# innate2adaptive/decombinator

Measured on AMD Instinct MI355X. Metric: Mreads/s decombined (150 bp human-beta), higher is better.
Workload: dtype u8

## Files before the change

decombinator_amd/csrc/dcrx_kernels_v2.hip:

```cpp
#include <hip/hip_runtime.h>
#include <hip/hip_ext.h>

#include <algorithm>
#include <cstddef>
#include <cstdio>
#include <cstdlib>
#include <vector>

#include "../../include/dcrx.h"
#include "dcrx_device.h"
#include "dcrx_launch.h"
#include "dcrx_dcr_device.h"
#include "dcrx_v2_device.h"
#include "dcrx_sink_device.h"

namespace dcrx {

bool first_use_on_device(bool (&seen)[64]);
void attributes_set_on_device(bool (&seen)[64]);

constexpr int DCRX_V2_BLOCK = 1024;
#ifdef DCRX_SCAN_STAMPS
__device__ uint32_t *g_scan_stamps;
#endif
constexpr int DCRX_V2_FBLOCK = 256;
#ifndef DCRX_V2_TBLOCK
#define DCRX_V2_TBLOCK 256
#define DCRX_V2_TWAVES 5
#endif
// ... 12 lines not shown
#define DCRX_STORE_SCAN dcrx_store_record_cached
#else
#define DCRX_STORE_SCAN dcrx_store_record
#endif
#ifndef DCRX_V2_LOOP_PRIO
#define DCRX_V2_LOOP_PRIO 2
#endif
#ifndef DCRX_V2_FULL_LINE_RECORDS
#define DCRX_V2_FULL_LINE_RECORDS 1
#endif
#ifndef DCRX_V2_ROLE_CALLS
#define DCRX_V2_ROLE_CALLS 0
#endif
#if DCRX_V2_ROLE_CALLS
#define DCRX_V2_ROLE __device__ __attribute__((noinline))
#else
#define DCRX_V2_ROLE __device__ __forceinline__
#endif
#ifndef DCRX_LEAN_LDS_WORDS
#define DCRX_LEAN_LDS_WORDS 1
#endif
constexpr uint32_t DCRX_V2_GROUP_MAX = 64;

enum { V2_L_TAIL = 0, V2_L_E = 1, V2_L_C = 2, V2_L_X = 3, V2_L_RING = 4, V2_L_TICKETS = 5, V2_L_TWHINT = 6, V2_L_COUNTS = 8 };
constexpr uint32_t V2_LEFT_CAP = 1024;
enum { V2_QC_LEFT = 5, V2_QC_DONE = 6 };
struct V2Lists {
  uint4 *tail;
  uint4 *ev;
  uint4 *sx;
  uint4 *left;
  uint32_t *counts;
  uint32_t tcap, ecap, scap;
};
template <int NW>
struct V2Rows {
  static constexpr int T = (2 + NW + 3) / 4, E = (1 + 2 * NW + 3) / 4;
  static_assert((2 + 2 * NW + 3) / 4 == E, "the digest word of an event entry (put_event) lies in the entry's last row");
};
struct V2ListRef { uint4 *rows; uint32_t cap; };
template <int NW>
__device__ __forceinline__ V2ListRef v2_list(const V2Lists &Q, const int which, const size_t region) {
  constexpr size_t E = V2Rows<NW>::E;
  if (which == V2_L_E) return V2ListRef{Q.ev + region * Q.ecap * E, Q.ecap};
  return V2ListRef{Q.sx + (region * Q.scap + (which == V2_L_X ? Q.scap / 2 : 0u)) * E, Q.scap / 2};
}
template <int N>
// ... 162 lines not shown
  for (uint64_t i = (uint64_t)e_lo + (uint32_t)tid; i < e_hi; i += blockDim.x) {
    const uint32_t r = B.exc_read[i];
    if (set) { if (i == e_lo || B.exc_read[i - 1] != r) atomicOr(&flag[r >> 5], 1u << (r & 31)); }
    else flag[r >> 5] = 0u;
  }
}

template <int NW>
__device__ __forceinline__ uint32_t *v2_left_valid(uint4 *left_rows) { return reinterpret_cast<uint32_t *>(left_rows + (size_t)V2_LEFT_CAP * V2Rows<NW>::E); }
template <int NW>
__device__ __forceinline__ bool v2_left_push(uint4 *left_rows, uint32_t *__restrict__ queue_count, const uint32_t x0, const uint32_t (&lg)[NW], const uint32_t (&w)[NW]) {
  const uint32_t at = atomicAdd(queue_count + V2_QC_LEFT, 1u);
  if (at >= V2_LEFT_CAP) return false;
  uint32_t x[1 + 2 * NW];
  x[0] = x0;
#pragma unroll
  for (int k = 0; k < NW; k++) { x[1 + k] = lg[k]; x[1 + NW + k] = w[k]; }
  v2_put_rows<1 + 2 * NW>(left_rows, 0u, at, x);
  __threadfence();
  __hip_atomic_store(v2_left_valid<NW>(left_rows) + at, 1u, __ATOMIC_RELAXED, __HIP_MEMORY_SCOPE_AGENT);
  return true;
}

enum { V2_WK_NEXT = 0, V2_WK_LIST = 1, V2_WK_EXC = 8, V2_WK_HEAD = 16, V2_WK_CLAIM = 17, V2_WK_SCANNED = 18, V2_WK_SINK = 19, V2_WK_HEAD2 = 20, V2_WK_CLAIM2 = 21,
       V2_WK_FILLED = 32, V2_WK_GEN = 48, V2_WK_FILLED2 = 64, V2_WK_GEN2 = 80, V2_WK_WORDS = 96 };
#ifndef DCRX_V2_FUSE_TAILWAVES
#define DCRX_V2_FUSE_TAILWAVES 3
#endif
#ifndef DCRX_V2_PRIO_TAIL
#define DCRX_V2_PRIO_TAIL 1
#endif
constexpr int V2_FUSE_TAILWAVES = DCRX_V2_FUSE_TAILWAVES;
constexpr uint32_t V2_TW6_FRAC256 = 243, V2_TW5_FRAC256 = 205, V2_TW4_FRAC256 = 136, V2_TW3_FRAC256 = 64;
constexpr int V2_RING_STRIDE = 15;
constexpr uint32_t V2_RING_MAXBATCHES = 16;
template <int NW> constexpr int v2_ering_stride() { return (2 * NW + 4) | 1; }
constexpr uint32_t V2_ERING_BATCHES = 8;
#ifndef DCRX_V2_HELP_DRAIN
#define DCRX_V2_HELP_DRAIN 0
#endif
constexpr float V2_FUSE_E_MAX_SHARE = 0.25f;

template <bool UNIFORM_LEN, int NW, int RPL, bool NARROW, bool PREFETCH = true, int FUSE = -1, bool SINK = false, bool FUSE_E = false>
__global__ __launch_bounds__(DCRX_V2_BLOCK) void scan2_kernel(
    DevTables T0, BatchDev B, CfgDev cfg, dcrx_record_t *__restrict__ records, unsigned long long *__restrict__ counters,
    V2Lists Q, uint32_t *__restrict__ queue, uint32_t *__restrict__ gqueue, uint32_t qcap, uint32_t *__restrict__ queue_count,
    uint64_t per_block, uint32_t retry, const DevTables *__restrict__ Tmem, uint32_t ring_batches, V2SinkCall S, uint32_t tail_waves, uint32_t rescue_waves) {
  static_assert(!FUSE_E || (FUSE >= 0 && !SINK), "the event ring rides on the fused form, without a tuple sink");
  extern __shared__ __align__(64) uint32_t smem[];
  if constexpr (FUSE >= 0 && !SINK) S.dev = nullptr;
  const int o = FUSE >= 0 ? FUSE : (cfg.orientation == DCRX_ORIENT_FORWARD ? 0 : 1);
  V2Ori V0 = T0.v2[0];
  if (o) V0 = T0.v2[1];
  uint32_t *lds_trans = smem;
  uint32_t *lds_counts = smem + V0.trans_bytes / 4;
  uint32_t *lds_work = lds_counts + DCRX_N_COUNTERS;
  const int tid = threadIdx.x;
#ifdef DCRX_SCAN_STAMPS
  const unsigned long long stamp_r0 = __builtin_amdgcn_s_memrealtime();
  unsigned long long stamp_setup = 0, stamp_loop_end = 0;
#endif
  if (tid < DCRX_N_COUNTERS) lds_counts[tid] = 0;
  if (tid < V2_WK_WORDS) lds_work[tid] = 0;
  {
    const uint4 *src = reinterpret_cast<const uint4 *>(V0.trans);
    uint4 *dst = reinterpret_cast<uint4 *>(lds_trans);
    for (uint32_t i = tid; i < V0.trans_bytes / 16; i += blockDim.x) dst[i] = src[i];
  }
  const V2Tab tab{};
  uint32_t *lds_side = lds_work + V2_WK_WORDS;
  uint32_t *lds_bk = lds_side + (T0.lds_image_bytes - T0.dfa_bytes) / 4;
  uint32_t *ring = lds_bk + V0.bk_bytes / 4;
  const uint32_t ring_mask = 64u * ring_batches - 1u;
  constexpr uint32_t ES = (uint32_t)v2_ering_stride<NW>(), ering_mask = 64u * V2_ERING_BATCHES - 1u;
  uint32_t *ring2 = ring + (size_t)(ring_mask + 1u) * V2_RING_STRIDE;
  uint32_t *lds_dry = ring2 + (size_t)(ering_mask + 1u) * ES;
  if (FUSE >= 0) {
    {
      const uint4 *s1 = reinterpret_cast<const uint4 *>(T0.image + T0.dfa_bytes), *s2 = reinterpret_cast<const uint4 *>(V0.bk);
      uint4 *d1 = reinterpret_cast<uint4 *>(lds_side), *d2 = reinterpret_cast<uint4 *>(lds_bk);
      for (uint32_t i = tid; i < (T0.lds_image_bytes - T0.dfa_bytes) / 16; i += blockDim.x) d1[i] = s1[i];
      for (uint32_t i = tid; i < V0.bk_bytes / 16; i += blockDim.x) d2[i] = s2[i];
    }
    for (uint32_t i = tid; i <= ring_mask; i += blockDim.x) { ring[i * V2_RING_STRIDE + NW] = 0u; ring[i * V2_RING_STRIDE + NW + 1] = 0u; }
    if (FUSE_E) for (uint32_t i = tid; i <= ering_mask; i += blockDim.x) { ring2[i * ES + NW] = 0u; ring2[i * ES + NW + 1] = 0u; }
  }
  __syncthreads();
  const uint32_t nw = B.stride >> 2;
  const int lane = tid & 63;
  const unsigned long long lt_mask = (1ull << lane) - 1ull;
  const bool tagged = B.n_reads < (1ull << 30);

  const uint64_t blk_lo = (uint64_t)blockIdx.x * per_block;
  const uint64_t blk_hi = blk_lo + per_block < B.n_reads ? blk_lo + per_block : B.n_reads;
  uint32_t e_lo = 0u, e_hi = 0u;
  if (B.n_exc) {
    v2_exc_slice(B, blk_lo < blk_hi ? blk_lo : blk_hi, blk_hi, lds_work + V2_WK_EXC, tid);
    e_lo = lds_work[V2_WK_EXC]; e_hi = lds_work[V2_WK_EXC + 2];
    v2_exc_marks(B, e_lo, e_hi, true, tid);
    asm volatile("s_waitcnt vmcnt(0)" ::: "memory");
    __syncthreads();
  }
  uint32_t tw = tail_waves;
  if (FUSE >= 0 && tw == 0u) {
    const uint32_t h = Q.counts[V2_L_COUNTS * blockIdx.x + V2_L_TWHINT + (o ? 0 : 1)];
    tw = (h >= 2u && h <= 8u) ? h : (uint32_t)V2_FUSE_TAILWAVES;
    if (FUSE_E && tw > 2u) tw -= 1u;
  }
// ... 103 lines not shown
        base = (uint32_t)__builtin_amdgcn_readfirstlane((int)base);
        const uint32_t at = base + (uint32_t)__popcll(mt0 & lt_mask);
        if (to_tail && at >= Q.tcap) { v2_hand_over(B, queue, gqueue, qcap, queue_count, tagged, (uint32_t)r, false); to_tail = false; }
        if (to_tail) {
          uint32_t x[2 + NW];
          x[0] = (uint32_t)r; x[1] = tail2_pack(d);
#pragma unroll
          for (int k = 0; k < NW; k++) x[2 + k] = w[q][k];
          v2_put_rows<2 + NW>(tq, Q.tcap, at, x);
        }
      }
      int lst = 0;
      if (what == V2_EVENTS) lst = (exc || bnd) ? V2_L_X : (shape2(d.vf_n, d.jf_n, d.any) == V2_SHAPE_BOTH ? V2_L_C : V2_L_E);
      auto put_event = [&](uint4 *rows, const uint32_t at) {
        uint32_t x[2 + 2 * NW];
        x[0] = (uint32_t)r | (exc ? V2_R_EXC : 0u);
#pragma unroll
        for (int k = 0; k < NW; k++) { x[1 + k] = lg[q][k]; x[1 + NW + k] = w[q][k]; }
        x[1 + 2 * NW] = rescue2_digest_pack(d);
        v2_put_rows<2 + 2 * NW>(rows, 0u, at, x);
      };
      bool to_ev = lst == V2_L_E;
      const unsigned long long me0 = __ballot(to_ev);
      if (FUSE_E) {
        if (me0) {
          constexpr uint32_t nb_mask = V2_ERING_BATCHES - 1u, nb_shift = (uint32_t)__builtin_ctz(V2_ERING_BATCHES);
          const uint32_t total = (uint32_t)__popcll(me0);
          const uint32_t genv = __hip_atomic_load(&lds_work[V2_WK_GEN2 + ((uint32_t)lane & nb_mask)], __ATOMIC_RELAXED, __HIP_MEMORY_SCOPE_WORKGROUP);
          uint32_t base = 0;
          if (lane == 0) base = atomicAdd(&lds_work[V2_WK_HEAD2], total);
          base = (uint32_t)__builtin_amdgcn_readfirstlane((int)base);
          const uint32_t gb0 = base >> 6, gbl = (base + total - 1u) >> 6;
          bool room = true;
          for (uint32_t g = gb0; g <= gbl; g++) room = room && (uint32_t)__builtin_amdgcn_readlane((int)genv, (int)(g & nb_mask)) >= (g >> nb_shift);
          if (!room && lane == 0) {
            bool ok = false;
            for (uint32_t spins = 0; spins < (1u << 24) && !ok; spins++) {
              ok = true;
              for (uint32_t g = gb0; g <= gbl; g++)
                ok = ok && __hip_atomic_load(&lds_work[V2_WK_GEN2 + (g & nb_mask)], __ATOMIC_RELAXED, __HIP_MEMORY_SCOPE_WORKGROUP) >= (g >> nb_shift);
              if (!ok) __builtin_amdgcn_s_sleep(2);
            }
            if (!ok) atomicAdd(&counters[DCRX_C_DEVICE_ERRORS], 1ull);
          }
          asm volatile("" ::: "memory");
          if (to_ev) {
            uint32_t *sl = ring2 + ((base + (uint32_t)__popcll(me0 & lt_mask)) & ering_mask) * ES;
#pragma unroll
            for (int k = 0; k < NW; k++) { sl[k] = w[q][k]; sl[NW + 3 + k] = lg[q][k]; }
            sl[NW + 2] = (uint32_t)r; sl[2 * NW + 3] = rescue2_digest_pack(d);
          }
          asm volatile("" ::: "memory");
          if (lane == 0) {
            for (uint32_t g = gb0; g <= gbl; g++) {
              const uint32_t lo = max(base, g << 6), hi = min(base + total, (g + 1u) << 6);
              atomicAdd(&lds_work[V2_WK_FILLED2 + (g & nb_mask)], hi - lo);
            }
          }
        }
      } else if (me0) {
        uint32_t base = 0;
        if (lane == 0) base = atomicAdd(&lds_work[V2_WK_LIST + V2_L_E], (uint32_t)__popcll(me0));
        base = (uint32_t)__builtin_amdgcn_readfirstlane((int)base);
        const uint32_t at = base + (uint32_t)__popcll(me0 & lt_mask);
        if (to_ev && at >= Q.ecap) {
          v2_hand_over(B, queue, gqueue, qcap, queue_count, tagged, (uint32_t)r, exc);
          to_ev = false;
        }
        if (to_ev) put_event(eq, at);
      }
      if (__ballot(lst > V2_L_E)) {
#pragma unroll 1
        for (int which = V2_L_C; which <= V2_L_X; which++) {
          const bool mine = lst == which;
          const unsigned long long mr = __ballot(mine);
          if (!mr) continue;
          uint32_t base = 0;
          if (lane == 0) base = atomicAdd(&lds_work[V2_WK_LIST + which], (uint32_t)__popcll(mr));
          base = (uint32_t)__builtin_amdgcn_readfirstlane((int)base);
          if (mine) {
            const V2ListRef l = v2_list<NW>(Q, which, region);
// ... 55 lines not shown
        for (int k = 0; k < NW; k++) w[q][k] = wn[q][k];
        xm[q] = xn[q];
      }
    }
    item = next;
  }
  if (FUSE >= 0 && lane == 0) {
    asm volatile("s_waitcnt lgkmcnt(0)" ::: "memory");
    atomicAdd(&lds_work[V2_WK_SCANNED], 1u);
  }
  }
  if (FUSE_E && (wv >= n_scan_waves + tw || (DCRX_V2_HELP_DRAIN && scans))) {
   if constexpr (FUSE_E) {
    constexpr bool REV = FUSE == 1;
#if DCRX_V2_PRIO_TAIL
    __builtin_amdgcn_s_setprio(DCRX_V2_PRIO_TAIL);
#endif
    uint32_t kw_base[K_NCLASS];
#pragma unroll
    for (int c = 0; c < K_NCLASS; c++) kw_base[c] = T0.kw_base[c];
    const Rescue2Tabs rt = rescue2_tabs(T0, V0, reinterpret_cast<const uint8_t *>(lds_side), reinterpret_cast<const uint8_t *>(lds_bk), REV, kw_base);
    const Counters C{lds_counts}, Cdry{lds_dry};
    constexpr uint32_t nb_mask = V2_ERING_BATCHES - 1u, nb_shift = (uint32_t)__builtin_ctz(V2_ERING_BATCHES);
    constexpr uint32_t V2_RING_EXIT = 0xFFFFFFFFu;
    for (uint32_t spins = 0;;) {
      uint32_t c = 0, nvalid = 0;
      if (lane == 0) {
        c = __hip_atomic_load(&lds_work[V2_WK_CLAIM2], __ATOMIC_RELAXED, __HIP_MEMORY_SCOPE_WORKGROUP);
        const bool mine = __hip_atomic_load(&lds_work[V2_WK_GEN2 + (c & nb_mask)], __ATOMIC_RELAXED, __HIP_MEMORY_SCOPE_WORKGROUP) == (c >> nb_shift);
        const uint32_t f = __hip_atomic_load(&lds_work[V2_WK_FILLED2 + (c & nb_mask)], __ATOMIC_RELAXED, __HIP_MEMORY_SCOPE_WORKGROUP);
        if (!mine) nvalid = 0;
        else if (f == 64u) nvalid = 64u;
        else if (__hip_atomic_load(&lds_work[V2_WK_SCANNED], __ATOMIC_RELAXED, __HIP_MEMORY_SCOPE_WORKGROUP) == n_scan_waves) {
          const uint32_t h = __hip_atomic_load(&lds_work[V2_WK_HEAD2], __ATOMIC_RELAXED, __HIP_MEMORY_SCOPE_WORKGROUP);
          const uint32_t rem = h - 64u * c;
          nvalid = (int32_t)rem <= 0 ? V2_RING_EXIT : min(rem, 64u);
        }
        if (nvalid && nvalid != V2_RING_EXIT) {
          uint32_t expect = c;
          if (!__hip_atomic_compare_exchange_strong(&lds_work[V2_WK_CLAIM2], &expect, c + 1u, __ATOMIC_RELAXED, __ATOMIC_RELAXED, __HIP_MEMORY_SCOPE_WORKGROUP)) nvalid = 0;
        }
      }
      c = (uint32_t)__builtin_amdgcn_readfirstlane((int)c);
      nvalid = (uint32_t)__builtin_amdgcn_readfirstlane((int)nvalid);
      if (nvalid == V2_RING_EXIT) break;
      if (!nvalid) {
        if (++spins > (1u << 24)) { if (lane == 0) atomicAdd(&counters[DCRX_C_DEVICE_ERRORS], 1ull); break; }
        __builtin_amdgcn_s_sleep(4);
        continue;
      }
      asm volatile("s_waitcnt lgkmcnt(0)" ::: "memory");
      uint32_t *sl = ring2 + ((64u * c + (uint32_t)lane) & ering_mask) * ES;
      int status = -2;
      uint32_t errs = 0, x0 = 0;
      uint32_t lg[NW];
#pragma unroll
      for (int k = 0; k < NW; k++) lg[k] = 0u;
      if ((uint32_t)lane < nvalid) {
        x0 = sl[NW + 2];
#pragma unroll
        for (int k = 0; k < NW; k++) lg[k] = sl[NW + 3 + k];
        const uint32_t dg = sl[2 * NW + 3];
        const uint32_t r = x0 & V2_R_MASK;
        const int n = UNIFORM_LEN ? (int)B.read_len : (int)B.lens[r];
        const LdsWords lw{dcrx_ldsaddr_of(sl)};
        auto on_ok = [&](dcrx_record_t rec, const uint32_t) {
          rec.frame = (uint8_t)(o ? 0 : 1);
          DCRX_STORE_FINISH(records + r, rec);
        };
        status = rescue2_fast_to<REV, NW, V2_SHAPE_ONE>(rt, lw, lg, n, cfg, on_ok, errs, *Tmem, C, Cdry, dg);
        if (status > 0) {
          dcrx_record_t rec;
          rec.v = rec.j = rec.v_start = rec.j_end = rec.ins_start = rec.ins_len = 0; rec.vdel = rec.jdel = 0;
          rec.status = (uint8_t)status; rec.frame = (uint8_t)(o ? 0 : 1);
          DCRX_STORE_FINISH(records + r, rec);
        } else if (status < 0) errs = 0;
      }
      v2_tally_rescue(lds_counts, lane, status, errs, o == 0);
      if (__builtin_expect(status == RESCUE2_SLOW, 0)) {
        uint32_t ww[NW];
#pragma unroll
        for (int k = 0; k < NW; k++) ww[k] = sl[k];
        if (!v2_left_push<NW>(Q.left, queue_count, x0, lg, ww)) v2_hand_over(B, queue, gqueue, qcap, queue_count, tagged, x0 & V2_R_MASK, false);
      }
      asm volatile("s_waitcnt lgkmcnt(0)" ::: "memory");
      if (lane == 0) {
        __hip_atomic_store(&lds_work[V2_WK_FILLED2 + (c & nb_mask)], 0u, __ATOMIC_RELAXED, __HIP_MEMORY_SCOPE_WORKGROUP);
        asm volatile("s_waitcnt lgkmcnt(0)" ::: "memory");
        atomicAdd(&lds_work[V2_WK_GEN2 + (c & nb_mask)], 1u);
      }
      spins = 0;
    }
   }
  }
  if (FUSE >= 0 && (DCRX_V2_HELP_DRAIN || (wv >= n_scan_waves && wv < n_scan_waves + tw))) {
   if constexpr (FUSE >= 0) {
    constexpr bool REV = FUSE == 1;
#if DCRX_V2_PRIO_TAIL
    __builtin_amdgcn_s_setprio(DCRX_V2_PRIO_TAIL);
#endif
    const Tail2Tabs tt = tail2_tabs(T0, V0, reinterpret_cast<const uint8_t *>(lds_side), reinterpret_cast<const uint8_t *>(lds_bk), REV);
    const Counters C{lds_counts};
    const uint32_t nb_mask = ring_batches - 1u, nb_shift = (uint32_t)__builtin_ctz(ring_batches);
    constexpr uint32_t V2_RING_EXIT = 0xFFFFFFFFu;
    for (uint32_t spins = 0;;) {
      uint32_t c = 0, nvalid = 0;
      if (lane == 0) {
        c = __hip_atomic_load(&lds_work[V2_WK_CLAIM], __ATOMIC_RELAXED, __HIP_MEMORY_SCOPE_WORKGROUP);
        const bool mine = __hip_atomic_load(&lds_work[V2_WK_GEN + (c & nb_mask)], __ATOMIC_RELAXED, __HIP_MEMORY_SCOPE_WORKGROUP) == (c >> nb_shift);
        const uint32_t f = __hip_atomic_load(&lds_work[V2_WK_FILLED + (c & nb_mask)], __ATOMIC_RELAXED, __HIP_MEMORY_SCOPE_WORKGROUP);
        if (!mine) nvalid = 0;
        else if (f == 64u) nvalid = 64u;
        else if (__hip_atomic_load(&lds_work[V2_WK_SCANNED], __ATOMIC_RELAXED, __HIP_MEMORY_SCOPE_WORKGROUP) == n_scan_waves) {
// ... 57 lines not shown
        __hip_atomic_store(&lds_work[V2_WK_FILLED + (c & nb_mask)], 0u, __ATOMIC_RELAXED, __HIP_MEMORY_SCOPE_WORKGROUP);
        asm volatile("s_waitcnt lgkmcnt(0)" ::: "memory");
        atomicAdd(&lds_work[V2_WK_GEN + (c & nb_mask)], 1u);
      }
      spins = 0;
    }
   }
  }
#ifdef DCRX_SCAN_STAMPS
  stamp_loop_end = __builtin_amdgcn_s_memrealtime();
#endif
  __syncthreads();
  if (B.n_exc) v2_exc_marks(B, e_lo, e_hi, false, tid);
#ifdef DCRX_SCAN_STAMPS
  if (lane == 0) {
    uint32_t *c = g_scan_stamps + 4 * ((size_t)blockIdx.x * (DCRX_V2_BLOCK / 64) + (size_t)(tid >> 6));
    c[0] = (uint32_t)stamp_r0; c[1] = (uint32_t)stamp_setup; c[2] = (uint32_t)stamp_loop_end; c[3] = (uint32_t)__builtin_amdgcn_s_memrealtime();
  }
#else
  if (tid < V2_L_COUNTS) {
    uint32_t c = tid <= V2_L_X ? lds_work[V2_WK_LIST + tid] : 0u;
    c = min(c, tid == V2_L_TAIL ? Q.tcap : (tid == V2_L_E ? Q.ecap : Q.scap / 2));
    if (tid == V2_L_RING) c = lds_work[V2_WK_HEAD];
    if ((tid == V2_L_TWHINT || tid == V2_L_TWHINT + 1) && FUSE >= 0) c = Q.counts[V2_L_COUNTS * region + tid];
    if (tid == V2_L_TWHINT + (o ? 0 : 1) && FUSE >= 0 && blk_hi > blk_lo) {
      const uint32_t frac256 = (uint32_t)(((uint64_t)lds_work[V2_WK_HEAD] << 8) / (blk_hi - blk_lo));
      c = frac256 >= V2_TW6_FRAC256 ? 6u : (frac256 >= V2_TW5_FRAC256 ? 5u : (frac256 >= V2_TW4_FRAC256 ? 4u : (frac256 >= V2_TW3_FRAC256 ? 3u : 2u)));
    }
    Q.counts[V2_L_COUNTS * region + tid] = c;
  }
  if (S.dev && tid == 0 && lds_work[V2_WK_SINK]) (void)__hip_atomic_fetch_add(S.hits + region, lds_work[V2_WK_SINK], __ATOMIC_RELAXED, __HIP_MEMORY_SCOPE_AGENT);
#endif
  if (tid < DCRX_N_COUNTERS && lds_counts[tid]) atomicAdd(&counters[tid], (unsigned long long)lds_counts[tid]);
}

static uint32_t v2_finish_lds_bytes(const DevTables &T, int o) {
  return DCRX_N_COUNTERS * 4 + (T.lds_image_bytes - T.dfa_bytes) + T.v2[o].bk_bytes;
}

template <bool UNIFORM_LEN, int NW, int ORI>
__device__ __forceinline__ void v2_general_entry(const DevTables &T, const V2Ori &V, const BatchDev &B, const CfgDev &cfg, const uint32_t x0,
                                                 const uint32_t (&lg)[NW], const uint32_t (&w)[NW], const Counters &C, dcrx_record_t *__restrict__ records,
                                                 uint32_t *__restrict__ queue, uint32_t *__restrict__ gqueue, const uint32_t qcap,
                                                 uint32_t *__restrict__ queue_count, const bool tagged) {
  const uint32_t r = x0 & V2_R_MASK;
  const bool exc = (x0 & V2_R_EXC) != 0u;
// ... 849 lines not shown
  Q.scap = (uint32_t)std::min<uint64_t>(Q.ecap, P.v2_slow_rows / V2Rows<NW>::E / n_regions) & ~127u;
  if (!ring_batches && (!P.v2_tail || Q.tcap < 64)) return B.n_reads ? hipErrorNotReady : hipSuccess;
  if (ring_batches) Q.tcap = (uint32_t)pb128 & ~63u;
  if (Q.ecap < 128 || Q.scap < 128) return hipErrorInvalidValue;
  const bool finish = !(cfg.flags & (DCRX_F_PROFILE_SCAN_ONLY | DCRX_F_PROFILE_NO_FINISH));
  const bool separate = (cfg.flags & (DCRX_F_V2_SIDE_STREAMS | DCRX_F_V2_LEAN_SERIAL | DCRX_F_V2_NO_LEAN_RESCUE)) != 0u;
  const bool side = finish && (cfg.flags & DCRX_F_V2_SIDE_STREAMS) && !(cfg.flags & DCRX_F_V2_LEAN_SERIAL) && P.v2_side && P.v2_side2 && P.v2_ev_fork &&
                    P.v2_ev_join && P.v2_ev_join2;
  const hipEvent_t fork_ev = ev_stop ? ev_stop : P.v2_ev_fork;
  static const uint32_t tail_waves_forced = [] { const char *e = dcrx_debug_env("DCRX_DEBUG_TAIL_WAVES"); const int v = e ? atoi(e) : 0; return (v >= 2 && v <= 8) ? (uint32_t)v : 0u; }();
  V2SinkCall S{};
  if (CAN_SINK && sink && P.sink.dev && finish && !separate && !retry && !(cfg.flags & DCRX_F_PROFILE_MASK)) {
    const uint64_t stride = (uint64_t)Q.tcap + Q.ecap + Q.scap / 2 + pb128;
    if (n_regions <= P.sink.regions_cap && stride * n_regions <= P.sink.items_cap && stride < (1ull << 32) && per_block / 32 * 8 <= 144u * 1024u &&
        per_block < 0xFFFFFFull) {
      S.dev = P.sink.dev; S.items = P.sink.items; S.hits = P.sink.hits; S.stride = (uint32_t)stride; S.e_off = Q.tcap; S.c_off = Q.tcap + Q.ecap; S.late_off = Q.tcap + Q.ecap + Q.scap / 2;
      S.late_cap = (uint32_t)pb128; S.per_block = (uint32_t)per_block; S.wpack = P.sink.wpack;
      sink->S = S; sink->n_regions = n_regions; sink->tcap = Q.tcap; sink->ecap = Q.ecap; sink->ccap = Q.scap / 2; sink->fused = ring_batches ? 1u : 0u;
      sink->counts = Q.counts;
    }
  }
  if (S.dev) fuse_e = false;
  if (P.tune && fuse_e) P.tune[o].last_form = 4u;
  static const uint32_t scan_threads = [] { const char *e = dcrx_debug_env("DCRX_DEBUG_SCAN_THREADS"); const int v = e ? atoi(e) : 0; return (v >= 512 && v <= DCRX_V2_BLOCK && v % 64 == 0) ? (uint32_t)v : (uint32_t)DCRX_V2_BLOCK; }();
  hipExtLaunchKernelGGL(S.dev ? ks_sink : (fuse_e ? ks_e : ks), dim3(grid), dim3(scan_threads), fuse_e ? scan_lds_e : scan_lds, s, ev_start ? ev_start : e_ev_start, side ? fork_ev : ev_stop, 0, T, B, cfg, rec,
                        d_counters, Q, queue, gqueue, qcap, queue_count, per_block, retry, P.dev_tables, fuse_e ? ring_batches_e : ring_batches, S, tail_waves_forced,
                        fuse_e ? rescue_waves_fused : 0u);
  e = hipGetLastError();
  if (e != hipSuccess) return e;
  if constexpr (CAN_FUSE_E) {
    if (eslot && eslot->fuse_e == -1 && !eslot->e_sampling && !fuse_e && fuse_e_env < 0 && !S.dev && finish) {
      bool ok = eslot->h_counts || eslot->h_counts.alloc((size_t)4096 * V2_L_COUNTS) == DCRX_OK;
      ok = ok && (eslot->ev_counts || eslot->ev_counts.create(false) == DCRX_OK);
      ok = ok && grid <= 4096u && hipMemcpyAsync(eslot->h_counts, Q.counts, (size_t)grid * V2_L_COUNTS * 4, hipMemcpyDeviceToHost, s) == hipSuccess &&
           hipEventRecord(eslot->ev_counts, s) == hipSuccess;
      if (ok) { eslot->e_sampling = true; eslot->e_regions = grid; eslot->e_reads = B.n_reads; }
      else { (void)hipGetLastError(); eslot->fuse_e = 0; }
    }
  }
  if (finish) {
    static const uint32_t rescue_waves_env = [] { const char *e = dcrx_debug_env("DCRX_DEBUG_RESCUE_WAVES"); const int v = e ? atoi(e) : 0; return v >= 256 ? (uint32_t)v : 0u; }();
    const bool big = B.n_reads >= V2Tune::BIG_BATCH;
    const uint32_t waves_first = (ring_batches && !separate && big) ? 8192u : 4096u, waves_second = (ring_batches && !separate && big) ? 4096u : 3072u;
    uint32_t rescue_waves = rescue_waves_env ? rescue_waves_env : ((ring_batches || separate) ? waves_first : (big ? 4096u : 3072u));
    hipEvent_t tune_start = nullptr, tune_stop = nullptr;
    static const bool tune_off = dcrx_debug_env("DCRX_DEBUG_NO_TUNE") != nullptr;
    const int tune_class = V2Tune::size_class(B.n_reads);
    if (ring_batches && !separate && !rescue_waves_env && !tune_off && P.tune && !retry && !cfg.flags && tune_class >= 0) {
      V2TuneSlot &U = P.tune[o].slot[tune_class];
      if (U.choice) rescue_waves = U.choice;
// ... 19 lines not shown
            for (int i = 0; i < V2Tune::SAMPLES && ok; i++) {
              float t = 0.f;
              ok = hipEventElapsedTime(&t, U.ev[i][0], U.ev[i][1]) == hipSuccess;
              ms[i & 1] += t;
            }
            (void)hipGetLastError();
            U.choice = (ok && ms[1] < 0.985f * ms[0]) ? waves_second : waves_first;
            if (ok) { U.us[0] = 1e3f * ms[0] / (V2Tune::SAMPLES / 2); U.us[1] = 1e3f * ms[1] / (V2Tune::SAMPLES / 2); }
            rescue_waves = U.choice;
            static const bool say = dcrx_debug_env("DCRX_DEBUG_TUNE") != nullptr;
            if (say) fprintf(stderr, "dcrx tune: finishing launches of %llu reads, frame %d: %.1f us on %u rescue waves, %.1f on %u -> %u (launch %d)\n",
                             (unsigned long long)B.n_reads, o, 1e3f * ms[0] / (V2Tune::SAMPLES / 2), waves_first, 1e3f * ms[1] / (V2Tune::SAMPLES / 2), waves_second, U.choice, U.launches);
          }
        }
        U.launches++;
      }
    }
    static const uint32_t tail_role_waves_env = [] { const char *e = dcrx_debug_env("DCRX_DEBUG_TAIL_ROLE_WAVES"); const int v = e ? atoi(e) : 0; return v >= 256 ? (uint32_t)v : 0u; }();
    const uint32_t tail_role_waves = tail_role_waves_env ? tail_role_waves_env : (separate ? 8192u : 4096u);
    const uint32_t tsplit = std::max<uint32_t>(1u, std::min<uint32_t>(64u, tail_role_waves / n_regions));
    const uint32_t rsplit_full = std::max<uint32_t>(1u, std::min<uint32_t>(64u, rescue_waves / n_regions));
    const uint32_t rsplit = fuse_e ? 1u : rsplit_full;
    static const uint32_t rescue_waves_c = [] { const char *e = dcrx_debug_env("DCRX_DEBUG_RESCUE_WAVES_C"); const int v = e ? atoi(e) : 0; return v >= 256 ? (uint32_t)v : 0u; }();
    const uint32_t csplit = rescue_waves_c ? std::max<uint32_t>(1u, std::min<uint32_t>(64u, rescue_waves_c / n_regions)) : rsplit_full;
    const uint32_t fgrid = (n_regions * (rsplit + csplit) + DCRX_V2_FBLOCK / 64 - 1) / (DCRX_V2_FBLOCK / 64);
    const uint32_t egrid = (n_regions + DCRX_V2_FBLOCK / 64 - 1) / (DCRX_V2_FBLOCK / 64);
    static const uint32_t bsplit_env = [] { const char *e = dcrx_debug_env("DCRX_DEBUG_X_BSPLIT"); const int v = e ? atoi(e) : 0; return (v >= 1 && v <= 16) ? (uint32_t)v : 0u; }();
    const uint32_t bsplit = bsplit_env ? bsplit_env : (separate ? std::max<uint32_t>(1u, std::min<uint32_t>(16u, 1024u / n_regions)) : (fuse_e ? 2u : 1u));
    const uint32_t sgrid = n_regions * bsplit;
    const uint32_t flds = v2_finish_lds_bytes(T, o);
    const uint32_t llds = v2_finish_block_lds<NW>(T, o, DCRX_V2_FBLOCK);
    const uint32_t tlds = v2_finish_block_lds<NW>(T, o, DCRX_V2_TBLOCK);
    const uint32_t elds_ext = flds + (T.lds_image2_bytes - T.lds_image_bytes);
    const uint32_t ext = elds_ext <= 64u * 1024u ? 1u : 0u;
    const uint32_t elds = ext ? elds_ext : flds;
    const uint32_t slow_width = 4u;
    const uint32_t tgrid = (n_regions * tsplit + DCRX_V2_TBLOCK / 64 - 1) / (DCRX_V2_TBLOCK / 64);
    V2Roles R;
    R.xgrid = sgrid; R.rgrid = fgrid; R.tgrid = ring_batches ? 0u : (n_regions * tsplit + DCRX_V2_FBLOCK / 64 - 1) / (DCRX_V2_FBLOCK / 64);
    R.rsplit = rsplit | (csplit << 8); R.tsplit = tsplit; R.bsplit = bsplit; R.width = slow_width;
    V2FinishArgs A;
    A.T0 = T; A.B = B; A.cfg = cfg; A.records = rec; A.counters = d_counters; A.Q = Q; A.n_regions = n_regions; A.R = R;
    A.queue = queue; A.gqueue = gqueue; A.qcap = qcap; A.queue_count = queue_count; A.Tmem = P.dev_tables; A.S = S;
    if (!separate) {
      hipExtLaunchKernelGGL(S.dev ? (ring_batches ? kf0_sink : kf_sink) : (ring_batches ? kf0 : kf), dim3(R.xgrid + R.rgrid + R.tgrid), dim3(DCRX_V2_FBLOCK), llds, s, tune_start,
                            tune_stop ? tune_stop : e_ev_stop, 0, A);
      e = hipGetLastError();
// ... 23 lines not shown
                           queue_count, P.dev_tables);
        e = hipGetLastError();
        if (e != hipSuccess) return e;
      }
      if (side) {
        e = hipStreamWaitEvent(s, P.v2_ev_join, 0); if (e != hipSuccess) return e;
        e = hipStreamWaitEvent(s, P.v2_ev_join2, 0); if (e != hipSuccess) return e;
      } else {
        hipLaunchKernelGGL(kt, dim3(tgrid), dim3(DCRX_V2_TBLOCK), tlds, s, T, B, cfg, rec, d_counters, Q, n_regions, tsplit, queue, gqueue, qcap, queue_count, P.dev_tables);
        e = hipGetLastError();
        if (e != hipSuccess) return e;
        e = general(s, V2_L_X, false, nullptr); if (e != hipSuccess) return e;
      }
      hipLaunchKernelGGL(kl, dim3(1), dim3(DCRX_V2_FBLOCK), llds, s, A);
      e = hipGetLastError(); if (e != hipSuccess) return e;
    }
    static const bool dbg = dcrx_debug_env("DCRX_DEBUG_V2_COUNTS") != nullptr;
    if (dbg && e == hipSuccess) {
      std::vector<uint32_t> h((size_t)V2_L_COUNTS * n_regions);
      (void)hipStreamSynchronize(s);
      (void)hipMemcpy(h.data(), Q.counts, h.size() * 4, hipMemcpyDeviceToHost);
      unsigned long long t[V2_L_COUNTS] = {0};
      for (uint32_t r = 0; r < n_regions; r++) for (int k = 0; k < V2_L_COUNTS; k++) t[k] += h[(size_t)V2_L_COUNTS * r + k];
      fprintf(stderr, "dcrx v2 lists: regions %u tail %llu E %llu C %llu X %llu; LDS of a finishing block %u bytes (side tables %u, buckets %u), of a scan block %u\n", n_regions,
              t[V2_L_TAIL], t[V2_L_E], t[V2_L_C], t[V2_L_X], llds, T.lds_image_bytes - T.dfa_bytes, T.v2[o].bk_bytes, scan_lds);
    }
  }
#ifdef DCRX_SCAN_STAMPS
  {
    static int launches = 0;
    static const int want = [] { const char *e = dcrx_debug_env("DCRX_STAMPS_LAUNCH"); return e ? atoi(e) : 30; }();
    if (launches++ == want && e == hipSuccess) {
      const size_t nw = (size_t)n_regions * (DCRX_V2_BLOCK / 64);
      std::vector<uint32_t> h(4 * nw);
      (void)hipStreamSynchronize(s);
      uint32_t *dptr = nullptr;
      (void)hipMemcpyFromSymbol(&dptr, HIP_SYMBOL(g_scan_stamps), sizeof(dptr));
      (void)hipMemcpy(h.data(), dptr, h.size() * 4, hipMemcpyDeviceToHost);
      if (const char *dump = dcrx_debug_env("DCRX_STAMPS_DUMP")) { FILE *f = fopen(dump, "wb"); if (f) { fwrite(h.data(), 4, h.size(), f); fclose(f); } }
      uint32_t t0 = 0xFFFFFFFFu;
      for (size_t i = 0; i < nw; i++) t0 = std::min(t0, h[4 * i]);
      auto pcs = [&](const char *what, std::vector<double> v) {
        std::sort(v.begin(), v.end());
        auto pc = [&](double q) { return v[(size_t)(q * (v.size() - 1))]; };
        fprintf(stderr, "dcrx scan stamps: %-44s min %6.1f p10 %6.1f p50 %6.1f p90 %6.1f p99 %6.1f max %6.1f us\n", what, pc(0), pc(0.1), pc(0.5), pc(0.9), pc(0.99), pc(1.0));
      };
      std::vector<double> st, su, le_scan, le_tail, en, blk_scan_end, blk_end;
      for (uint32_t r = 0; r < n_regions; r++) {
// ... 82 lines not shown
```

Measured before the change: 33370.

## Route list-C events through a second in-block LDS ring in the fused scan

Adds a second LDS ring (two batches) to the fused event form so that reads classified as list C (both V and J shapes) are handed to in-block rescue waves and finished with the two-shape rescue path, instead of being written to the global C list for a later finishing kernel. The rescue loop now prefers full C-ring batches and drains remaining C entries after the E ring is exhausted. The producer and consumer ring code is factored into generic lambdas, the C split of the finishing grid drops to one when the ring is on, and per-region counts gain a slot for the C-ring total. This is meant to cut global list traffic and finishing-kernel work for C events, at the cost of extra LDS per scan block (possibly lower occupancy) and more contention on the in-block rescue waves.

```diff
diff --git a/decombinator_amd/csrc/dcrx_kernels_v2.hip b/decombinator_amd/csrc/dcrx_kernels_v2.hip
--- a/decombinator_amd/csrc/dcrx_kernels_v2.hip
+++ b/decombinator_amd/csrc/dcrx_kernels_v2.hip
@@ -5,6 +5,7 @@
 #include <cstddef>
 #include <cstdio>
 #include <cstdlib>
+#include <type_traits>
 #include <vector>
 
 #include "../../include/dcrx.h"
@@ -63,7 +64,7 @@
 #endif
 constexpr uint32_t DCRX_V2_GROUP_MAX = 64;
 
-enum { V2_L_TAIL = 0, V2_L_E = 1, V2_L_C = 2, V2_L_X = 3, V2_L_RING = 4, V2_L_TICKETS = 5, V2_L_TWHINT = 6, V2_L_COUNTS = 8 };
+enum { V2_L_TAIL = 0, V2_L_E = 1, V2_L_C = 2, V2_L_X = 3, V2_L_RING = 4, V2_L_TICKETS = 5, V2_L_TWHINT = 6, V2_L_CRING = 8, V2_L_COUNTS = 10 };
 constexpr uint32_t V2_LEFT_CAP = 1024;
 enum { V2_QC_LEFT = 5, V2_QC_DONE = 6 };
 struct V2Lists {
@@ -272,8 +273,8 @@
   return true;
 }
 
-enum { V2_WK_NEXT = 0, V2_WK_LIST = 1, V2_WK_EXC = 8, V2_WK_HEAD = 16, V2_WK_CLAIM = 17, V2_WK_SCANNED = 18, V2_WK_SINK = 19, V2_WK_HEAD2 = 20, V2_WK_CLAIM2 = 21,
-       V2_WK_FILLED = 32, V2_WK_GEN = 48, V2_WK_FILLED2 = 64, V2_WK_GEN2 = 80, V2_WK_WORDS = 96 };
+enum { V2_WK_NEXT = 0, V2_WK_LIST = 1, V2_WK_EXC = 8, V2_WK_HEAD = 16, V2_WK_CLAIM = 17, V2_WK_SCANNED = 18, V2_WK_SINK = 19, V2_WK_HEAD2 = 20, V2_WK_CLAIM2 = 21, V2_WK_HEAD3 = 22, V2_WK_CLAIM3 = 23,
+       V2_WK_FILLED = 32, V2_WK_GEN = 48, V2_WK_FILLED2 = 64, V2_WK_FILLED3 = 72, V2_WK_GEN2 = 80, V2_WK_GEN3 = 88, V2_WK_WORDS = 96 };
 #ifndef DCRX_V2_FUSE_TAILWAVES
 #define DCRX_V2_FUSE_TAILWAVES 3
 #endif
@@ -286,6 +287,9 @@
 constexpr uint32_t V2_RING_MAXBATCHES = 16;
 template <int NW> constexpr int v2_ering_stride() { return (2 * NW + 4) | 1; }
 constexpr uint32_t V2_ERING_BATCHES = 8;
+constexpr uint32_t V2_CRING_BATCHES = 2;
+static_assert(V2_WK_FILLED2 + V2_ERING_BATCHES <= V2_WK_FILLED3 && V2_WK_FILLED3 + V2_CRING_BATCHES <= V2_WK_GEN2 && V2_WK_GEN2 + V2_ERING_BATCHES <= V2_WK_GEN3 &&
+              V2_WK_GEN3 + V2_CRING_BATCHES <= V2_WK_WORDS, "the rings' words do not overlap");
 #ifndef DCRX_V2_HELP_DRAIN
 #define DCRX_V2_HELP_DRAIN 0
 #endif
@@ -295,7 +299,7 @@
 __global__ __launch_bounds__(DCRX_V2_BLOCK) void scan2_kernel(
     DevTables T0, BatchDev B, CfgDev cfg, dcrx_record_t *__restrict__ records, unsigned long long *__restrict__ counters,
     V2Lists Q, uint32_t *__restrict__ queue, uint32_t *__restrict__ gqueue, uint32_t qcap, uint32_t *__restrict__ queue_count,
-    uint64_t per_block, uint32_t retry, const DevTables *__restrict__ Tmem, uint32_t ring_batches, V2SinkCall S, uint32_t tail_waves, uint32_t rescue_waves) {
+    uint64_t per_block, uint32_t retry, const DevTables *__restrict__ Tmem, uint32_t ring_batches, V2SinkCall S, uint32_t tail_waves, uint32_t rescue_waves, uint32_t c_ring) {
   static_assert(!FUSE_E || (FUSE >= 0 && !SINK), "the event ring rides on the fused form, without a tuple sink");
   extern __shared__ __align__(64) uint32_t smem[];
   if constexpr (FUSE >= 0 && !SINK) S.dev = nullptr;
@@ -324,7 +328,10 @@
   const uint32_t ring_mask = 64u * ring_batches - 1u;
   constexpr uint32_t ES = (uint32_t)v2_ering_stride<NW>(), ering_mask = 64u * V2_ERING_BATCHES - 1u;
   uint32_t *ring2 = ring + (size_t)(ring_mask + 1u) * V2_RING_STRIDE;
-  uint32_t *lds_dry = ring2 + (size_t)(ering_mask + 1u) * ES;
+  constexpr uint32_t cring_mask = 64u * V2_CRING_BATCHES - 1u;
+  uint32_t *ring3 = ring2 + (size_t)(ering_mask + 1u) * ES;
+  const bool cring = FUSE_E && c_ring != 0u;
+  uint32_t *lds_dry = ring3 + (cring ? (size_t)(cring_mask + 1u) * ES : (size_t)0);
   if (FUSE >= 0) {
     {
       const uint4 *s1 = reinterpret_cast<const uint4 *>(T0.image + T0.dfa_bytes), *s2 = reinterpret_cast<const uint4 *>(V0.bk);
@@ -333,7 +340,7 @@
       for (uint32_t i = tid; i < V0.bk_bytes / 16; i += blockDim.x) d2[i] = s2[i];
     }
     for (uint32_t i = tid; i <= ring_mask; i += blockDim.x) { ring[i * V2_RING_STRIDE + NW] = 0u; ring[i * V2_RING_STRIDE + NW + 1] = 0u; }
-    if (FUSE_E) for (uint32_t i = tid; i <= ering_mask; i += blockDim.x) { ring2[i * ES + NW] = 0u; ring2[i * ES + NW + 1] = 0u; }
+    if (FUSE_E) for (uint32_t i = tid; i <= ering_mask + (cring ? cring_mask + 1u : 0u); i += blockDim.x) { ring2[i * ES + NW] = 0u; ring2[i * ES + NW + 1] = 0u; }
   }
   __syncthreads();
   const uint32_t nw = B.stride >> 2;
@@ -483,41 +490,48 @@
       };
       bool to_ev = lst == V2_L_E;
       const unsigned long long me0 = __ballot(to_ev);
+      auto ring_put = [&](auto nbc, const unsigned long long m, const bool mine, uint32_t *rg, const int head, const int gen, const int filled) {
+        constexpr uint32_t NB = decltype(nbc)::value, nb_mask = NB - 1u, nb_shift = (uint32_t)__builtin_ctz(NB), rg_mask = 64u * NB - 1u;
+        const uint32_t total = (uint32_t)__popcll(m);
+        const uint32_t genv = __hip_atomic_load(&lds_work[gen + ((uint32_t)lane & nb_mask)], __ATOMIC_RELAXED, __HIP_MEMORY_SCOPE_WORKGROUP);
+        uint32_t base = 0;
+        if (lane == 0) base = atomicAdd(&lds_work[head], total);
+        base = (uint32_t)__builtin_amdgcn_readfirstlane((int)base);
+        const uint32_t gb0 = base >> 6, gbl = (base + total - 1u) >> 6;
+        bool room = true;
+        for (uint32_t g = gb0; g <= gbl; g++) room = room && (uint32_t)__builtin_amdgcn_readlane((int)genv, (int)(g & nb_mask)) >= (g >> nb_shift);
+        if (!room && lane == 0) {
+          bool ok = false;
+          for (uint32_t spins = 0; spins < (1u << 24) && !ok; spins++) {
+            ok = true;
+            for (uint32_t g = gb0; g <= gbl; g++)
+              ok = ok && __hip_atomic_load(&lds_work[gen + (g & nb_mask)], __ATOMIC_RELAXED, __HIP_MEMORY_SCOPE_WORKGROUP) >= (g >> nb_shift);
+            if (!ok) __builtin_amdgcn_s_sleep(2);
+          }
+          if (!ok) atomicAdd(&counters[DCRX_C_DEVICE_ERRORS], 1ull);
+        }
+        asm volatile("" ::: "memory");
+        if (mine) {
+          uint32_t *sl = rg + ((base + (uint32_t)__popcll(m & lt_mask)) & rg_mask) * ES;
+#pragma unroll
+          for (int k = 0; k < NW; k++) { sl[k] = w[q][k]; sl[NW + 3 + k] = lg[q][k]; }
+          sl[NW + 2] = (uint32_t)r; sl[2 * NW + 3] = rescue2_digest_pack(d);
+        }
+        asm volatile("" ::: "memory");
+        if (lane == 0) {
+          for (uint32_t g = gb0; g <= gbl; g++) {
+            const uint32_t lo = max(base, g << 6), hi = min(base + total, (g + 1u) << 6);
+            atomicAdd(&lds_work[filled + (g & nb_mask)], hi - lo);
+          }
+        }
+      };
       if (FUSE_E) {
-        if (me0) {
-          constexpr uint32_t nb_mask = V2_ERING_BATCHES - 1u, nb_shift = (uint32_t)__builtin_ctz(V2_ERING_BATCHES);
-          const uint32_t total = (uint32_t)__popcll(me0);
-          const uint32_t genv = __hip_atomic_load(&lds_work[V2_WK_GEN2 + ((uint32_t)lane & nb_mask)], __ATOMIC_RELAXED, __HIP_MEMORY_SCOPE_WORKGROUP);
-          uint32_t base = 0;
-          if (lane == 0) base = atomicAdd(&lds_work[V2_WK_HEAD2], total);
-          base = (uint32_t)__builtin_amdgcn_readfirstlane((int)base);
-          const uint32_t gb0 = base >> 6, gbl = (base + total - 1u) >> 6;
-          bool room = true;
-          for (uint32_t g = gb0; g <= gbl; g++) room = room && (uint32_t)__builtin_amdgcn_readlane((int)genv, (int)(g & nb_mask)) >= (g >> nb_shift);
-          if (!room && lane == 0) {
-            bool ok = false;
-            for (uint32_t spins = 0; spins < (1u << 24) && !ok; spins++) {
-              ok = true;
-              for (uint32_t g = gb0; g <= gbl; g++)
-                ok = ok && __hip_atomic_load(&lds_work[V2_WK_GEN2 + (g & nb_mask)], __ATOMIC_RELAXED, __HIP_MEMORY_SCOPE_WORKGROUP) >= (g >> nb_shift);
-              if (!ok) __builtin_amdgcn_s_sleep(2);
-            }
-            if (!ok) atomicAdd(&counters[DCRX_C_DEVICE_ERRORS], 1ull);
-          }
-          asm volatile("" ::: "memory");
-          if (to_ev) {
-            uint32_t *sl = ring2 + ((base + (uint32_t)__popcll(me0 & lt_mask)) & ering_mask) * ES;
-#pragma unroll
-            for (int k = 0; k < NW; k++) { sl[k] = w[q][k]; sl[NW + 3 + k] = lg[q][k]; }
-            sl[NW + 2] = (uint32_t)r; sl[2 * NW + 3] = rescue2_digest_pack(d);
-          }
-          asm volatile("" ::: "memory");
-          if (lane == 0) {
-            for (uint32_t g = gb0; g <= gbl; g++) {
-              const uint32_t lo = max(base, g << 6), hi = min(base + total, (g + 1u) << 6);
-              atomicAdd(&lds_work[V2_WK_FILLED2 + (g & nb_mask)], hi - lo);
-            }
-          }
+        if (me0) ring_put(std::integral_constant<uint32_t, V2_ERING_BATCHES>{}, me0, to_ev, ring2, V2_WK_HEAD2, V2_WK_GEN2, V2_WK_FILLED2);
+        if (cring) {
+          const bool to_c = lst == V2_L_C;
+          const unsigned long long mc0 = __ballot(to_c);
+          if (mc0) ring_put(std::integral_constant<uint32_t, V2_CRING_BATCHES>{}, mc0, to_c, ring3, V2_WK_HEAD3, V2_WK_GEN3, V2_WK_FILLED3);
+          if (to_c) lst = 0;
         }
       } else if (me0) {
         uint32_t base = 0;
@@ -619,35 +633,11 @@
     const Rescue2Tabs rt = rescue2_tabs(T0, V0, reinterpret_cast<const uint8_t *>(lds_side), reinterpret_cast<const uint8_t *>(lds_bk), REV, kw_base);
     const Counters C{lds_counts}, Cdry{lds_dry};
     constexpr uint32_t nb_mask = V2_ERING_BATCHES - 1u, nb_shift = (uint32_t)__builtin_ctz(V2_ERING_BATCHES);
+    constexpr uint32_t cb_mask = V2_CRING_BATCHES - 1u, cb_shift = (uint32_t)__builtin_ctz(V2_CRING_BATCHES);
     constexpr uint32_t V2_RING_EXIT = 0xFFFFFFFFu;
-    for (uint32_t spins = 0;;) {
-      uint32_t c = 0, nvalid = 0;
-      if (lane == 0) {
-        c = __hip_atomic_load(&lds_work[V2_WK_CLAIM2], __ATOMIC_RELAXED, __HIP_MEMORY_SCOPE_WORKGROUP);
-        const bool mine = __hip_atomic_load(&lds_work[V2_WK_GEN2 + (c & nb_mask)], __ATOMIC_RELAXED, __HIP_MEMORY_SCOPE_WORKGROUP) == (c >> nb_shift);
-        const uint32_t f = __hip_atomic_load(&lds_work[V2_WK_FILLED2 + (c & nb_mask)], __ATOMIC_RELAXED, __HIP_MEMORY_SCOPE_WORKGROUP);
-        if (!mine) nvalid = 0;
-        else if (f == 64u) nvalid = 64u;
-        else if (__hip_atomic_load(&lds_work[V2_WK_SCANNED], __ATOMIC_RELAXED, __HIP_MEMORY_SCOPE_WORKGROUP) == n_scan_waves) {
-          const uint32_t h = __hip_atomic_load(&lds_work[V2_WK_HEAD2], __ATOMIC_RELAXED, __HIP_MEMORY_SCOPE_WORKGROUP);
-          const uint32_t rem = h - 64u * c;
-          nvalid = (int32_t)rem <= 0 ? V2_RING_EXIT : min(rem, 64u);
-        }
-        if (nvalid && nvalid != V2_RING_EXIT) {
-          uint32_t expect = c;
-          if (!__hip_atomic_compare_exchange_strong(&lds_work[V2_WK_CLAIM2], &expect, c + 1u, __ATOMIC_RELAXED, __ATOMIC_RELAXED, __HIP_MEMORY_SCOPE_WORKGROUP)) nvalid = 0;
-        }
-      }
-      c = (uint32_t)__builtin_amdgcn_readfirstlane((int)c);
-      nvalid = (uint32_t)__builtin_amdgcn_readfirstlane((int)nvalid);
-      if (nvalid == V2_RING_EXIT) break;
-      if (!nvalid) {
-        if (++spins > (1u << 24)) { if (lane == 0) atomicAdd(&counters[DCRX_C_DEVICE_ERRORS], 1ull); break; }
-        __builtin_amdgcn_s_sleep(4);
-        continue;
-      }
+    auto batch = [&](auto shape, uint32_t *rg, const uint32_t rg_mask, const uint32_t c, const uint32_t nvalid, uint32_t *filled, uint32_t *gen) {
       asm volatile("s_waitcnt lgkmcnt(0)" ::: "memory");
-      uint32_t *sl = ring2 + ((64u * c + (uint32_t)lane) & ering_mask) * ES;
+      uint32_t *sl = rg + ((64u * c + (uint32_t)lane) & rg_mask) * ES;
       int status = -2;
       uint32_t errs = 0, x0 = 0;
       uint32_t lg[NW];
@@ -665,7 +655,7 @@
           rec.frame = (uint8_t)(o ? 0 : 1);
           DCRX_STORE_FINISH(records + r, rec);
         };
-        status = rescue2_fast_to<REV, NW, V2_SHAPE_ONE>(rt, lw, lg, n, cfg, on_ok, errs, *Tmem, C, Cdry, dg);
+        status = rescue2_fast_to<REV, NW, decltype(shape)::value>(rt, lw, lg, n, cfg, on_ok, errs, *Tmem, C, Cdry, dg);
         if (status > 0) {
           dcrx_record_t rec;
           rec.v = rec.j = rec.v_start = rec.j_end = rec.ins_start = rec.ins_len = 0; rec.vdel = rec.jdel = 0;
@@ -682,10 +672,54 @@
       }
       asm volatile("s_waitcnt lgkmcnt(0)" ::: "memory");
       if (lane == 0) {
-        __hip_atomic_store(&lds_work[V2_WK_FILLED2 + (c & nb_mask)], 0u, __ATOMIC_RELAXED, __HIP_MEMORY_SCOPE_WORKGROUP);
+        __hip_atomic_store(filled, 0u, __ATOMIC_RELAXED, __HIP_MEMORY_SCOPE_WORKGROUP);
         asm volatile("s_waitcnt lgkmcnt(0)" ::: "memory");
-        atomicAdd(&lds_work[V2_WK_GEN2 + (c & nb_mask)], 1u);
-      }
+        atomicAdd(gen, 1u);
+      }
+    };
+    for (uint32_t spins = 0;;) {
+      uint32_t c = 0, nvalid = 0, from_c = 0;
+      if (lane == 0) {
+        uint32_t c3 = 0;
+        bool mine3 = false;
+        if (cring) {
+          c3 = __hip_atomic_load(&lds_work[V2_WK_CLAIM3], __ATOMIC_RELAXED, __HIP_MEMORY_SCOPE_WORKGROUP);
+          mine3 = __hip_atomic_load(&lds_work[V2_WK_GEN3 + (c3 & cb_mask)], __ATOMIC_RELAXED, __HIP_MEMORY_SCOPE_WORKGROUP) == (c3 >> cb_shift);
+          if (mine3 && __hip_atomic_load(&lds_work[V2_WK_FILLED3 + (c3 & cb_mask)], __ATOMIC_RELAXED, __HIP_MEMORY_SCOPE_WORKGROUP) == 64u) { from_c = 1u; c = c3; nvalid = 64u; }
+        }
+        if (!from_c) {
+          c = __hip_atomic_load(&lds_work[V2_WK_CLAIM2], __ATOMIC_RELAXED, __HIP_MEMORY_SCOPE_WORKGROUP);
+          const bool mine = __hip_atomic_load(&lds_work[V2_WK_GEN2 + (c & nb_mask)], __ATOMIC_RELAXED, __HIP_MEMORY_SCOPE_WORKGROUP) == (c >> nb_shift);
+          const uint32_t f = __hip_atomic_load(&lds_work[V2_WK_FILLED2 + (c & nb_mask)], __ATOMIC_RELAXED, __HIP_MEMORY_SCOPE_WORKGROUP);
+          if (!mine) nvalid = 0;
+          else if (f == 64u) nvalid = 64u;
+          else if (__hip_atomic_load(&lds_work[V2_WK_SCANNED], __ATOMIC_RELAXED, __HIP_MEMORY_SCOPE_WORKGROUP) == n_scan_waves) {
+            const uint32_t h = __hip_atomic_load(&lds_work[V2_WK_HEAD2], __ATOMIC_RELAXED, __HIP_MEMORY_SCOPE_WORKGROUP);
+            const uint32_t rem = h - 64u * c;
+            nvalid = (int32_t)rem <= 0 ? V2_RING_EXIT : min(rem, 64u);
+          }
+          if (cring && nvalid == V2_RING_EXIT) {
+            const uint32_t h3 = __hip_atomic_load(&lds_work[V2_WK_HEAD3], __ATOMIC_RELAXED, __HIP_MEMORY_SCOPE_WORKGROUP);
+            const uint32_t rem3 = h3 - 64u * c3;
+            if ((int32_t)rem3 > 0) { from_c = 1u; c = c3; nvalid = mine3 ? min(rem3, 64u) : 0u; }
+          }
+        }
+        if (nvalid && nvalid != V2_RING_EXIT) {
+          uint32_t expect = c;
+          if (!__hip_atomic_compare_exchange_strong(&lds_work[from_c ? V2_WK_CLAIM3 : V2_WK_CLAIM2], &expect, c + 1u, __ATOMIC_RELAXED, __ATOMIC_RELAXED, __HIP_MEMORY_SCOPE_WORKGROUP)) nvalid = 0;
+        }
+      }
+      c = (uint32_t)__builtin_amdgcn_readfirstlane((int)c);
+      nvalid = (uint32_t)__builtin_amdgcn_readfirstlane((int)nvalid);
+      from_c = (uint32_t)__builtin_amdgcn_readfirstlane((int)from_c);
+      if (nvalid == V2_RING_EXIT) break;
+      if (!nvalid) {
+        if (++spins > (1u << 24)) { if (lane == 0) atomicAdd(&counters[DCRX_C_DEVICE_ERRORS], 1ull); break; }
+        __builtin_amdgcn_s_sleep(4);
+        continue;
+      }
+      if (from_c) batch(std::integral_constant<int, V2_SHAPE_BOTH>{}, ring3, cring_mask, c, nvalid, &lds_work[V2_WK_FILLED3 + (c & cb_mask)], &lds_work[V2_WK_GEN3 + (c & cb_mask)]);
+      else batch(std::integral_constant<int, V2_SHAPE_ONE>{}, ring2, ering_mask, c, nvalid, &lds_work[V2_WK_FILLED2 + (c & nb_mask)], &lds_work[V2_WK_GEN2 + (c & nb_mask)]);
       spins = 0;
     }
    }
@@ -789,6 +823,7 @@
     uint32_t c = tid <= V2_L_X ? lds_work[V2_WK_LIST + tid] : 0u;
     c = min(c, tid == V2_L_TAIL ? Q.tcap : (tid == V2_L_E ? Q.ecap : Q.scap / 2));
     if (tid == V2_L_RING) c = lds_work[V2_WK_HEAD];
+    if (tid == V2_L_CRING) c = FUSE_E ? lds_work[V2_WK_HEAD3] : 0u;
     if ((tid == V2_L_TWHINT || tid == V2_L_TWHINT + 1) && FUSE >= 0) c = Q.counts[V2_L_COUNTS * region + tid];
     if (tid == V2_L_TWHINT + (o ? 0 : 1) && FUSE >= 0 && blk_hi > blk_lo) {
       const uint32_t frac256 = (uint32_t)(((uint64_t)lds_work[V2_WK_HEAD] << 8) / (blk_hi - blk_lo));
@@ -1684,10 +1719,13 @@
   }
   if (S.dev) fuse_e = false;
   if (P.tune && fuse_e) P.tune[o].last_form = 4u;
+  const uint32_t cring_bytes = 64u * V2_CRING_BATCHES * (uint32_t)v2_ering_stride<NW>() * 4u;
+  const uint32_t c_ring = (fuse_e && scan_lds_e + cring_bytes <= 160u * 1024u) ? 1u : 0u;
+  if (c_ring) scan_lds_e += cring_bytes;
   static const uint32_t scan_threads = [] { const char *e = dcrx_debug_env("DCRX_DEBUG_SCAN_THREADS"); const int v = e ? atoi(e) : 0; return (v >= 512 && v <= DCRX_V2_BLOCK && v % 64 == 0) ? (uint32_t)v : (uint32_t)DCRX_V2_BLOCK; }();
   hipExtLaunchKernelGGL(S.dev ? ks_sink : (fuse_e ? ks_e : ks), dim3(grid), dim3(scan_threads), fuse_e ? scan_lds_e : scan_lds, s, ev_start ? ev_start : e_ev_start, side ? fork_ev : ev_stop, 0, T, B, cfg, rec,
                         d_counters, Q, queue, gqueue, qcap, queue_count, per_block, retry, P.dev_tables, fuse_e ? ring_batches_e : ring_batches, S, tail_waves_forced,
-                        fuse_e ? rescue_waves_fused : 0u);
+                        fuse_e ? rescue_waves_fused : 0u, c_ring);
   e = hipGetLastError();
   if (e != hipSuccess) return e;
   if constexpr (CAN_FUSE_E) {
@@ -1753,7 +1791,7 @@
     const uint32_t rsplit_full = std::max<uint32_t>(1u, std::min<uint32_t>(64u, rescue_waves / n_regions));
     const uint32_t rsplit = fuse_e ? 1u : rsplit_full;
     static const uint32_t rescue_waves_c = [] { const char *e = dcrx_debug_env("DCRX_DEBUG_RESCUE_WAVES_C"); const int v = e ? atoi(e) : 0; return v >= 256 ? (uint32_t)v : 0u; }();
-    const uint32_t csplit = rescue_waves_c ? std::max<uint32_t>(1u, std::min<uint32_t>(64u, rescue_waves_c / n_regions)) : rsplit_full;
+    const uint32_t csplit = c_ring ? 1u : (rescue_waves_c ? std::max<uint32_t>(1u, std::min<uint32_t>(64u, rescue_waves_c / n_regions)) : rsplit_full);
     const uint32_t fgrid = (n_regions * (rsplit + csplit) + DCRX_V2_FBLOCK / 64 - 1) / (DCRX_V2_FBLOCK / 64);
     const uint32_t egrid = (n_regions + DCRX_V2_FBLOCK / 64 - 1) / (DCRX_V2_FBLOCK / 64);
     static const uint32_t bsplit_env = [] { const char *e = dcrx_debug_env("DCRX_DEBUG_X_BSPLIT"); const int v = e ? atoi(e) : 0; return (v >= 1 && v <= 16) ? (uint32_t)v : 0u; }();
@@ -1823,8 +1861,8 @@
       (void)hipMemcpy(h.data(), Q.counts, h.size() * 4, hipMemcpyDeviceToHost);
       unsigned long long t[V2_L_COUNTS] = {0};
       for (uint32_t r = 0; r < n_regions; r++) for (int k = 0; k < V2_L_COUNTS; k++) t[k] += h[(size_t)V2_L_COUNTS * r + k];
-      fprintf(stderr, "dcrx v2 lists: regions %u tail %llu E %llu C %llu X %llu; LDS of a finishing block %u bytes (side tables %u, buckets %u), of a scan block %u\n", n_regions,
-              t[V2_L_TAIL], t[V2_L_E], t[V2_L_C], t[V2_L_X], llds, T.lds_image_bytes - T.dfa_bytes, T.v2[o].bk_bytes, scan_lds);
+      fprintf(stderr, "dcrx v2 lists: regions %u tail %llu E %llu C %llu X %llu, through list C's ring %llu; LDS of a finishing block %u bytes (side tables %u, buckets %u), of a scan block %u\n", n_regions,
+              t[V2_L_TAIL], t[V2_L_E], t[V2_L_C], t[V2_L_X], t[V2_L_CRING], llds, T.lds_image_bytes - T.dfa_bytes, T.v2[o].bk_bytes, fuse_e ? scan_lds_e : scan_lds);
     }
   }
 #ifdef DCRX_SCAN_STAMPS
```

New measurement: 32230. 3.4% lower.
